# miemie2013/Pytorch-PPYOLO

Measured on AMD Instinct MI355X. Metric: images/sec PPYOLO R50-vd 608x608 bs=8, higher is better.
Workload: dtype f32; 1 GPU; PPYOLO ResNet50-vd (DCNv2, CoordConv, SPP) 608x608, 8 images per GPU, device-resident input -> padded detections; global_batch=8, parallelism=single GPU, hip_graph=True, tile_table=tuned_gfx950_f16x2.json

## Files before the change

include/ppyolo_hip.h:

```cpp
#ifndef PPYOLO_HIP_H_
#define PPYOLO_HIP_H_

#include <stddef.h>
#include <stdint.h>

#ifdef __cplusplus
extern "C" {
#endif

#define PPY_OK 0
#define PPY_ERR_BAD_ARG (-1)
#define PPY_ERR_UNSUPPORTED (-2)
#define PPY_ERR_WORKSPACE (-3)
#define PPY_ERR_LAUNCH (-4)

#define PPY_ACT_NONE 0
#define PPY_ACT_RELU 1
#define PPY_ACT_LEAKY 2

int ppy_version(void);
const char *ppy_error_string(int code);
const char *ppy_last_hip_error(void);
void ppy_note_hip_error(int hip_error);

// ... 161 lines not shown

int ppy_yolo_decode_levels_f32(int nlevels, const float *const *head_out, const int *head_ld, const int *S,
                               const int *downsample, const float *const *h_anchors_px,
                               const int *box_offset, int N, int A, int num_classes, double scale_x_y,
                               int iou_aware, double iou_aware_factor, int clip_bbox, const float *im_size,
                               float *boxes, int M_total, float score_threshold, uint32_t *cand_key,
                               uint32_t *cand_idx, int *cand_count, int cand_cap, void *stream);

size_t ppy_matrix_nms_workspace_bytes(int N);
int ppy_matrix_nms_f32(const float *boxes, int M_total, int num_classes, const uint32_t *cand_key,
                       const uint32_t *cand_idx, const int *cand_count, int cand_cap, int N,
                       float post_threshold, int nms_top_k, int keep_top_k, int use_gaussian,
                       float gaussian_sigma, float *out_dets, int *out_count, int *out_keep_idx,
                       void *ws, size_t ws_bytes, void *stream);
int ppy_nms_candidates_f32(const float *scores, int N, int M, int C, float score_threshold,
                           uint32_t *cand_key, uint32_t *cand_idx, int *cand_count, int cand_cap,
                           void *stream);

int ppy_conv3x3_conv1x1_f32(const float *x_split, int x_ld, const float *xscale, const float *amax_in, const void *wA_f16x2,
                            const float *scaleA_f16x2, const float *shiftA, const void *wB_f16x2, const float *scaleB_f16x2,
                            const float *shiftB, const float *residual, int res_ld, float *y, int y_ld, float *pool, int pool_ld, int N,
                            int H, int W, int CA, int KA, int KB, float t_mul, float t_add, float *amax_out, void *stream);

int ppy_lane_stream_create(void **stream, const uint32_t *h_cu_mask, int mask_words);
int ppy_lane_stream_destroy(void *stream);

#ifdef __cplusplus
}
#endif
#endif
```

pytorch-ppyolo_amd/ppyolo_hip/_lib.py:

```python
import ctypes
import os
from ctypes import c_double, c_float, c_int, c_longlong, c_size_t, c_ulonglong, c_void_p

_HERE = os.path.dirname(os.path.abspath(__file__))
LIB_PATH = os.environ.get('PPYOLO_HIP_LIB') or os.path.join(_HERE, 'lib', 'libppyolo_hip.so')

OK = 0
ACT = {None: 0, 'relu': 1, 'leaky': 2}


class PPYoloHipError(RuntimeError):
    pass


_lib = None

_PROTOS = {
    'ppy_version': (c_int, []),
    'ppy_error_string': (ctypes.c_char_p, [c_int]),
    'ppy_last_hip_error': (ctypes.c_char_p, []),
    'ppy_note_hip_error': (None, [c_int]),
    'ppy_conv2d_split_weights_bf16x3': (c_int, [c_void_p, ctypes.c_longlong, c_void_p, c_void_p]),
    'ppy_conv2d_split_weights_f16x2': (c_int, [c_void_p, c_int, ctypes.c_longlong, c_void_p, c_void_p, c_void_p, c_void_p]),
    'ppy_conv2d_bn_act_f32': (c_int, [c_void_p, c_int, c_void_p, c_void_p, c_void_p, c_void_p, c_void_p, c_void_p, c_void_p,
# ... 65 lines not shown
                            c_void_p]),
    'ppy_dcnv2_sample_f32': (c_int, [c_void_p, c_int, c_void_p, c_int, c_void_p] + [c_int] * 8 + [c_void_p]),
    'ppy_dcnv2_f32': (c_int, [c_void_p, c_int, c_void_p, c_void_p, c_void_p, c_void_p, c_void_p, c_void_p, c_void_p, c_int,
                              c_void_p, c_int] + [c_int] * 10 + [c_void_p, c_void_p, c_void_p, c_size_t, c_void_p]),
    'ppy_dcnv2_workspace_bytes': (c_size_t, [c_int] * 9),
    'ppy_dcnv2_num_configs': (c_int, []),
    'ppy_dcnv2_backward_f32': (c_int, [c_void_p, c_int, c_void_p, c_void_p, c_int, c_void_p, c_int, c_void_p, c_int, c_void_p, c_int, c_void_p]
                               + [c_int] * 7 + [c_void_p, c_size_t, c_void_p]),
    'ppy_dcnv2_backward_workspace_bytes': (c_size_t, [c_int] * 7),
    'ppy_yolo_decode_f32': (c_int, [c_void_p, c_int, c_int, c_int, c_int, c_int, ctypes.POINTER(c_float), c_int,
                                    c_double, c_int, c_double, c_int, c_void_p, c_void_p, c_int, c_int, c_float,
                                    c_void_p, c_void_p, c_void_p, c_int, c_void_p, c_void_p]),
    'ppy_yolo_decode_levels_f32': (c_int, [c_int, c_void_p, c_void_p, c_void_p, c_void_p, c_void_p, c_void_p, c_int, c_int,
                                           c_int, c_double, c_int, c_double, c_int, c_void_p, c_void_p, c_int, c_float,
                                           c_void_p, c_void_p, c_void_p, c_int, c_void_p]),
    'ppy_matrix_nms_f32': (c_int, [c_void_p, c_int, c_int, c_void_p, c_void_p, c_void_p, c_int, c_int, c_float,
                                   c_int, c_int, c_int, c_float, c_void_p, c_void_p, c_void_p, c_void_p, c_size_t,
                                   c_void_p]),
    'ppy_matrix_nms_workspace_bytes': (c_size_t, [c_int]),
    'ppy_nms_candidates_f32': (c_int, [c_void_p, c_int, c_int, c_int, c_float, c_void_p, c_void_p, c_void_p,
                                       c_int, c_void_p]),
    'ppy_conv3x3_conv1x1_f32': (c_int, [c_void_p, c_int, c_void_p, c_void_p, c_void_p, c_void_p, c_void_p, c_void_p, c_void_p, c_void_p, c_void_p,
                                         c_int, c_void_p, c_int, c_void_p, c_int] + [c_int] * 6 + [c_float, c_float, c_void_p, c_void_p]),
    'ppy_lane_stream_create': (c_int, [ctypes.POINTER(c_void_p), ctypes.POINTER(ctypes.c_uint32), c_int]),
    'ppy_lane_stream_destroy': (c_int, [c_void_p]),
}


def exported_symbols():
    return sorted(_PROTOS)


def lib():
    global _lib
    if _lib is None:
        if not os.path.exists(LIB_PATH):
            raise PPYoloHipError(
                'libppyolo_hip.so not found at %s -- build it with `python -c "import __graft_entry__ as g; '
                'g.build()"` (hipcc, gfx950). There is no CPU / PyTorch fallback for the HIP path.' % LIB_PATH)
        import torch
        L = ctypes.CDLL(LIB_PATH)
        for name, (res, args) in _PROTOS.items():
            fn = getattr(L, name)
            fn.restype = res
            fn.argtypes = args
        _lib = L
# ... 10 lines not shown
```

pytorch-ppyolo_amd/ppyolo_hip/csrc/conv_b2b.hip:

```cpp
#include "conv_shared.h"

namespace {

struct B2bArgs {
    const float *x;
    const unsigned short *wA, *wB;
    const float *scaleA, *shiftA, *scaleB, *shiftB;
    const float *res;
    float *y;
    float *pool;
    const float *xscale;
    const float *amax_in;
    float *amax_out;
    float t_mul, t_add;
    int x_ld, res_ld, y_ld, pool_ld, N, H, W, M;
    int skip;
};

template <int CA, int KA, int KB, bool POOL>
__global__ void __launch_bounds__(256, 2) conv_b2b_kernel(const B2bArgs p) {
#if defined(__HIP_DEVICE_COMPILE__)
    constexpr int BM = 128, NW = 4;
    constexpr int TY = 8, TX = 16, WX = TX + 2, WPIX = (TY + 2) * WX;
    constexpr int TNA = KA / 32, HB = KB / 2, TNH = HB / 32;
    constexpr int CCH = CA / 32, NCH = 9 * CCH, KCH = KA / 32;
    constexpr int WIN_CC = WPIX * 128, WIN_BYTES = CCH * WIN_CC;
    constexpr int WIN_UNITS = CCH * WPIX * 8, WIN_PASS = (WIN_UNITS + 64 * NW - 1) / (64 * NW);
    constexpr int B_PASS = (2 * KA) / (16 * NW), G = B_PASS;
    constexpr int BST = 2 * KA * 64, BS_OFF = WIN_PASS * NW * 1024;
    constexpr int A2_BYTES = KCH * BM * 128;
    constexpr int W_OFF = A2_BYTES, W_BYTES = KCH * 2 * HB * 64;
    constexpr int E_OFF = W_OFF + W_BYTES;
    constexpr int B2_PASS = W_BYTES / (1024 * NW);
    static_assert(TY * TX == BM && TY == 2 * NW && TX == 16, "a wave owns two tile rows as eight 2x2 blocks");
    static_assert(KA % 32 == 0 && KB % 64 == 0 && CA % 32 == 0 && (2 * KA) % (16 * NW) == 0 && W_BYTES % (1024 * NW) == 0 && HB % 16 == 0, "shapes");
    static_assert(BS_OFF >= WIN_BYTES && BS_OFF + 3 * BST <= E_OFF + NW * 4096, "window + weight stages fit the allocation");
    typedef __attribute__((address_space(3))) void *lds_ptr;
    extern __shared__ __attribute__((aligned(16))) char smem_b2b[];
    char *smem = smem_b2b;

    const int tid = threadIdx.x, lane = tid & 63;
    const int wave = __builtin_amdgcn_readfirstlane(tid >> 6);
    int tile_id;
    {
        const int nb = (int)gridDim.x, q = nb >> 3, r = nb & 7;
        const int xcd = (int)blockIdx.x & 7, idx = (int)blockIdx.x >> 3;
        tile_id = xcd * q + min(xcd, r) + idx;
    }
    const int hw = p.H * p.W;
    const int tiles_x = (p.W + TX - 1) / TX, tiles_y = (p.H + TY - 1) / TY;
    const int t_n = tile_id / (tiles_x * tiles_y), t_rem = tile_id - t_n * (tiles_x * tiles_y);
    const int t_y = t_rem / tiles_x, t_x = t_rem - t_y * tiles_x;
    const int y0 = t_y * TY, x0 = t_x * TX;
    auto pixel_of = [&](int R) -> int {
        const int w = R >> 5, r = R & 31;
        const int y = y0 + 2 * w + (r >> 4), x = x0 + 2 * (r & 7) + ((r >> 3) & 1);
        return (y < p.H && x < p.W) ? t_n * hw + y * p.W + x : -1;
    };
    const unsigned OOB = 0xFFFFFFF0u;
    {
        const __amdgpu_buffer_rsrc_t rx = __builtin_amdgcn_make_buffer_rsrc((void *)p.x, 0, 0xFFFFFF00u, 0x00020000);
#pragma unroll
        for (int d = 0; d < WIN_PASS; ++d) {
            const int q = (d * NW + wave) * 64 + lane;
            const int pq = q >> 3, cc = pq / WPIX, wp = pq - cc * WPIX;
            const int wy = wp / WX, wx = wp - wy * WX;
            const int y = y0 - 1 + wy, x = x0 - 1 + wx;
            const bool ok = q < WIN_UNITS && (unsigned)y < (unsigned)p.H && (unsigned)x < (unsigned)p.W;
            const unsigned off = ok ? (unsigned)(((t_n * p.H + y) * p.W + x) * (p.x_ld * 4) + cc * 128 + (((q & 7) ^ ((wp >> 1) & 7)) << 4)) : OOB;
            __builtin_amdgcn_raw_ptr_buffer_load_lds(rx, (lds_ptr)(smem + (d * NW + wave) * 1024), 16, off, 0, 0, 0);
        }
    }
    unsigned b_off[B_PASS];
    {
        const int drow = lane >> 2, dslot = lane & 3;
        const long long plane_bytes = (long long)KA * (9 * CA) * 2;
#pragma unroll
        for (int j = 0; j < B_PASS; ++j) {
            const int rb = (j * NW + wave) * 16 + drow;
            const int plane = rb / KA, nrow = rb - plane * KA;
            const int scol = dslot ^ ((rb >> 2) & 3);
            b_off[j] = (unsigned)(plane * plane_bytes + (long long)nrow * 64 + scol * 16);
        }
    }
    const char *wb = reinterpret_cast<const char *>(p.wA);
    auto issue = [&](int stage, int kc) {
        const int cc = kc / 9, tap = kc - cc * 9;
        const long long b_uni = ((long long)tap * CCH + cc) * KA * 64;
        const __amdgpu_buffer_rsrc_t rb = __builtin_amdgcn_make_buffer_rsrc((void *)(wb + b_uni), 0, 0xFFFFFF00u, 0x00020000);
#pragma unroll
        for (int j = 0; j < B_PASS; ++j)
            __builtin_amdgcn_raw_ptr_buffer_load_lds(rb, (lds_ptr)(smem + BS_OFF + stage * BST + (j * NW + wave) * 1024), 16, b_off[j], 0, 0, 0);
    };

    const int frow = lane & 31, fkh = lane >> 5;
    const int wp0 = (2 * wave + (frow >> 4)) * WX + 2 * (frow & 7) + ((frow >> 3) & 1);
    const int a_sw = (frow >> 1) & 7, b_sw = (frow >> 2) & 3;
    int a_foff[2][2], b_foff[2];
#pragma unroll
    for (int s = 0; s < 2; ++s) {
        a_foff[s][0] = frow * 128 + (((2 * s + fkh) ^ a_sw) << 4);
        a_foff[s][1] = frow * 128 + (((4 + 2 * s + fkh) ^ a_sw) << 4);
        b_foff[s] = frow * 64 + (((2 * s + fkh) ^ b_sw) << 4);
    }

    float inv_sa, s2, inv_s2;
    {
        const int n = min(t_n, p.N - 1);
        inv_sa = pow2_inverse(p.xscale[n]);
        s2 = split_scale_of(fmaf(p.t_mul, pow2_above(amax_read(p.amax_in, n)), p.t_add));
        inv_s2 = pow2_inverse(s2);
    }
    issue(0, 0);
    issue(1, 1);
    const int erow = lane >> 3, ec4 = (lane & 7) * 4;
    int pix[4];
#pragma unroll
    for (int t = 0; t < 4; ++t) pix[t] = pixel_of(wave * 32 + erow + 8 * t);
    unsigned roff[4], yoff[4];
#pragma unroll
    for (int t = 0; t < 4; ++t) {
        roff[t] = ((unsigned)max(pix[t], 0) * (unsigned)p.res_ld + (unsigned)ec4) * 4u;
        yoff[t] = ((unsigned)max(pix[t], 0) * (unsigned)p.y_ld + (unsigned)ec4) * 4u;
    }
    const char *res_b = reinterpret_cast<const char *>(p.res);
    constexpr unsigned B2B_OOB = 0x80000000u;
    const __amdgpu_buffer_rsrc_t ry = __builtin_amdgcn_make_buffer_rsrc((void *)p.y, 0, B2B_OOB, 0x00020000);
    const __amdgpu_buffer_rsrc_t rp = __builtin_amdgcn_make_buffer_rsrc((void *)(POOL ? p.pool : p.y), 0, B2B_OOB, 0x00020000);
    const bool no_stores = (p.skip & 4) != 0;
#pragma unroll
    for (int t = 0; t < 4; ++t)
        if (pix[t] < 0 || no_stores) yoff[t] = B2B_OOB;
    floatx4 rv[TNH][4];
    auto load_res = [&](int col0, floatx4 (&dst)[4]) {
#pragma unroll
        for (int t = 0; t < 4; ++t)
            dst[t] = *reinterpret_cast<const floatx4 *>(res_b + (size_t)roff[t] + col0 * 4);
    };
#pragma unroll
    for (int jj = 0; jj < TNH; ++jj) load_res(jj * 32, rv[jj]);
    floatx16 acc[TNA];
#pragma unroll
    for (int j = 0; j < TNA; ++j)
#pragma unroll
        for (int e = 0; e < 16; ++e) acc[j][e] = 0.f;
    if (!(p.skip & 1))
    for (int k = 0; k < NCH; ++k) {
        if (k < 2 && (p.skip & 16))
            wait_vmcnt<0>();
        else if (k < 2)
            wait_vmcnt<G + 4 * TNH>();
        else if (k + 1 < NCH)
            wait_vmcnt<G>();
        else
            wait_vmcnt<0>();
        asm volatile("s_waitcnt lgkmcnt(0)" ::: "memory");
        __builtin_amdgcn_s_barrier();
        if (k + 2 < NCH) issue((k + 2) % 3, k + 2);
        const int st = k % 3;
        const int cc = k / 9, tap = k - cc * 9, tr = tap / 3;
        const int wp = wp0 + tr * WX + (tap - tr * 3);
        const char *a_ptr = smem + cc * WIN_CC + wp * 128;
        const int wsw = (wp >> 1) & 7;
        const char *b_ptr = smem + BS_OFF + st * BST;
#pragma unroll
        for (int s = 0; s < 2; ++s) {
            const uintx4 a0 = *reinterpret_cast<const uintx4 *>(a_ptr + (((2 * s + fkh) ^ wsw) << 4));
            const uintx4 a1 = *reinterpret_cast<const uintx4 *>(a_ptr + (((4 + 2 * s + fkh) ^ wsw) << 4));
            uintx4 b[2][TNA];
#pragma unroll
            for (int pl = 0; pl < 2; ++pl)
#pragma unroll
                for (int j = 0; j < TNA; ++j) b[pl][j] = *reinterpret_cast<const uintx4 *>(b_ptr + (pl * KA + j * 32) * 64 + b_foff[s]);
// ... 6 lines not shown
#pragma unroll
            for (int j = 0; j < TNA; ++j)
                acc[j] = __builtin_amdgcn_mfma_f32_32x32x16_f16(__builtin_bit_cast(f16x8, a0), __builtin_bit_cast(f16x8, b[0][j]), acc[j], 0, 0, 0);
        }
    }
    asm volatile("s_waitcnt lgkmcnt(0)" ::: "memory");
    __builtin_amdgcn_s_barrier();

    const __amdgpu_buffer_rsrc_t rw2 = __builtin_amdgcn_make_buffer_rsrc((void *)p.wB, 0, 0xFFFFFF00u, 0x00020000);
    auto issue_w2 = [&](int half) {
        const int drow = lane >> 2, dslot = lane & 3;
        const unsigned plane_bytes = (unsigned)KB * KA * 2;
#pragma unroll
        for (int j = 0; j < B2_PASS; ++j) {
            const int R = (j * NW + wave) * 16 + drow;
            const int blk = R / HB, r = R - blk * HB;
            const int scol = dslot ^ ((R >> 2) & 3);
            const unsigned off = (unsigned)(blk & 1) * plane_bytes + (unsigned)((blk >> 1) * KB * 64 + (half * HB + r) * 64 + scol * 16);
            __builtin_amdgcn_raw_ptr_buffer_load_lds(rw2, (lds_ptr)(smem + W_OFF + (j * NW + wave) * 1024), 16, off, 0, 0, 0);
        }
    };
    if (p.skip & 1) wait_vmcnt<0>();
    if (p.skip & 2) return;
    issue_w2(0);

    float *sE = reinterpret_cast<float *>(smem + E_OFF) + wave * 1024;
    {
        float rs1[4], rs2[4];
#pragma unroll
        for (int t = 0; t < 4; ++t) {
            rs1[t] = __shfl(inv_sa, (lane >> 3) + 8 * t);
            rs2[t] = __shfl(s2, (lane >> 3) + 8 * t);
        }
#pragma unroll
        for (int j = 0; j < TNA; ++j) {
            const int col = j * 32 + ec4;
            const floatx4 sc = *reinterpret_cast<const floatx4 *>(p.scaleA + col), sh = *reinterpret_cast<const floatx4 *>(p.shiftA + col);
#pragma unroll
            for (int e = 0; e < 16; ++e) {
                const int row = (e & 3) + 8 * (e >> 2) + 4 * (lane >> 5);
                sE[row * 32 + ((lane & 31) ^ ((row & 7) << 2))] = acc[j][e];
            }
            __builtin_amdgcn_wave_barrier();
#pragma unroll
            for (int t = 0; t < 4; ++t) {
                const int rr = erow + 8 * t;
// ... 115 lines not shown
                                       const float *shiftB, const float *residual, int res_ld, float *y, int y_ld, float *pool, int pool_ld,
                                       int N, int H, int W, int CA, int KA, int KB, float t_mul, float t_add, float *amax_out, void *stream) {
    ppy_drop_stale_error();
    PPY_CHECK_ARG(x_split && xscale && amax_in && wA_f16x2 && scaleA_f16x2 && shiftA && wB_f16x2 && scaleB_f16x2 && shiftB && residual && y);
    PPY_CHECK_ARG(N > 0 && H > 0 && W > 0 && t_mul >= 0.f && t_add >= 0.f);
    if (!(CA == 64 && KA == 64 && KB == 256)) return PPY_ERR_UNSUPPORTED;
    PPY_CHECK_ARG(x_ld >= CA && x_ld % 32 == 0 && res_ld >= KB && res_ld % 4 == 0 && y_ld >= KB && y_ld % 4 == 0);
    auto al = [](const void *q) { return ((uintptr_t)q & 15) == 0; };
    PPY_CHECK_ARG(al(x_split) && al(wA_f16x2) && al(wB_f16x2) && al(scaleA_f16x2) && al(shiftA) && al(scaleB_f16x2) && al(shiftB) && al(residual) && al(y));
    if (pool) PPY_CHECK_ARG(H % 2 == 0 && W % 2 == 0 && pool_ld >= KB && pool_ld % 4 == 0 && al(pool));
    const long long M = (long long)N * H * W;
    if (M > 0x7fffffffLL / 4 || (M + W + 1) * x_ld * 4 >= 0xFFFFF000LL || M * res_ld * 4 >= 0xFFFFF000LL || M * y_ld * 4 >= 0x7FFFF000LL ||
        (pool && (M / 4) * pool_ld * 4 >= 0x7FFFF000LL)) return PPY_ERR_UNSUPPORTED;
    B2bArgs a;
    a.x = x_split; a.wA = (const unsigned short *)wA_f16x2; a.wB = (const unsigned short *)wB_f16x2;
    a.scaleA = scaleA_f16x2; a.shiftA = shiftA; a.scaleB = scaleB_f16x2; a.shiftB = shiftB;
    a.res = residual; a.y = y; a.pool = pool; a.xscale = xscale; a.amax_in = amax_in; a.amax_out = amax_out;
    a.t_mul = t_mul; a.t_add = t_add;
    { static const int sk = getenv("PPY_B2B_SKIP") ? atoi(getenv("PPY_B2B_SKIP")) : 0; a.skip = sk; }
    a.x_ld = x_ld; a.res_ld = res_ld; a.y_ld = y_ld; a.pool_ld = pool_ld; a.N = N; a.H = H; a.W = W; a.M = (int)M;
    constexpr size_t lds = 2 * 128 * 128 + 2 * 2 * 128 * 64 + 4 * 4096;
    const unsigned grid = (unsigned)(N * ((H + 7) / 8) * ((W + 15) / 16));
    if (pool) {
        auto k = conv_b2b_kernel<64, 64, 256, true>;
        static PpyLdsAttr attr;
        if (ppy_lds_attr(attr, reinterpret_cast<const void *>(k), (int)lds) != PPY_OK) return PPY_ERR_LAUNCH;
        hipLaunchKernelGGL(k, dim3(grid), dim3(256), lds, (hipStream_t)stream, a);
    } else {
        auto k = conv_b2b_kernel<64, 64, 256, false>;
        static PpyLdsAttr attr;
        if (ppy_lds_attr(attr, reinterpret_cast<const void *>(k), (int)lds) != PPY_OK) return PPY_ERR_LAUNCH;
        hipLaunchKernelGGL(k, dim3(grid), dim3(256), lds, (hipStream_t)stream, a);
    }
    return ppy_launch_status();
}
```

pytorch-ppyolo_amd/ppyolo_hip/engine.py:

```python
import collections
import json
import os

import torch

from . import ops as K
from ._lib import PPYoloHipError

A = collections.namedtuple('A', 'buf coff C N H W')


def fold_bn(bn, bias, K_out, device):
    if bn is not None:
        invstd = 1.0 / torch.sqrt(bn.running_var.detach().float() + bn.eps)
        scale = bn.weight.detach().float() * invstd
        shift = bn.bias.detach().float() - bn.running_mean.detach().float() * scale
        if bias is not None:
            shift = shift + bias.detach().float() * scale
    else:
        scale = torch.ones(K_out, dtype=torch.float32, device=device)
        shift = bias.detach().float().clone() if bias is not None else torch.zeros(K_out, dtype=torch.float32,
                                                                                   device=device)
    return scale.contiguous(), shift.contiguous()

# ... 301 lines not shown
        for b in outs:
            writers.setdefault(b, []).append(op)
    out = []
    for a in ops:
        if a['op'] != 'conv' or not has_f16(a):
            continue
        Ka, R, S, Ca = a['w'].shape
        y = a['y']
        if (R, S, a['stride'], a['pad'], Ca, Ka, a['act']) != (3, 3, 1, 1, 64, 64, 'relu') or a['res'] is not None or a['posb'] is not None \
                or a['ups'] or a.get('pool') is not None or a.get('mpool') is not None or y.buf in pinned \
                or y.coff != 0 or y.C != buffers[y.buf][3] or len(writers.get(y.buf, [])) != 1:
            continue
        rd = readers.get(y.buf, [])
        if len(rd) != 1 or rd[0]['op'] != 'conv':
            continue
        b = rd[0]
        Kb, Rb, Sb, Cb = b['w'].shape
        x = b['x']
        if (Rb, Sb, b['stride'], b['pad'], Cb, Kb, b['act']) != (1, 1, 1, 0, 64, 256, 'relu') or b['res'] is None or b['posb'] is not None \
                or b['ups'] or not has_f16(b) or (x.buf, x.coff, x.C) != (y.buf, 0, 64) or b['res'].buf == y.buf \
                or b.get('stream', 0) != a.get('stream', 0):
            continue
        out.append((a, b))
    return out


class HipExecutor(object):

    def __init__(self, plan, device, use_graph=True, multi_stream=None, share=None):
        if torch.device(device).type != 'cuda':
            raise PPYoloHipError('the HIP executor needs a ROCm device (got %s); there is no CPU path' % device)
        self.plan = plan
        self.device = torch.device(device)
        self.use_graph = use_graph
        self.graph = None
        self._graph_stream = None
        p = plan
        self.bufs = None
        self.x_in = torch.zeros((p.N, 3, p.H, p.W), dtype=torch.float32, device=self.device)
        self.im_size = torch.zeros((p.N, 2), dtype=torch.float32, device=self.device)
        d = p.decode
        if d is not None:
            M, C = d['M_total'], d['num_classes']
            self.boxes = torch.zeros((p.N, M, 4), dtype=torch.float32, device=self.device)
            cap = M * C
            self.cand_key = torch.zeros((p.N, cap), dtype=torch.int32, device=self.device)
# ... 124 lines not shown
    def _split_pairs(self):
        if self.math != 'f16x2' or os.environ.get('PPYOLO_HIP_PRESPLIT', '1') != '1':
            return []
        pinned = {a.buf for a in list(self.plan.head_outs) + list(self.plan.feats)}
        return split_pairs(self.plan.ops, self._op_io, self.plan.buffers, pinned,
                           lambda c: c.get('wf16') is not None and c.get('amax_in_id') is not None,
                           os.environ.get('PPYOLO_HIP_PRESPLIT_3X3_ONLY', '0') == '1')

    def _mark_split_candidates(self):
        for op in self.plan.ops:
            op.pop('gp_in', None)
        for _, cons in self._split_pairs():
            for c in cons:
                c['gp_in'] = True

    def _unlink_splits(self):
        for op in self.plan.ops:
            op.pop('x_split', None)
            op.pop('y_split', None)

    def _link_splits(self, _retry=False):
        if not _retry:
            self._b2b_rejected = set()
        self._unlink_splits()
        self._mark_b2b()
        n = 0
        for pr, cons in self._split_pairs():
            if pr.get('b2b') is not None or pr.get('b2b_of') is not None:
                continue
            if self._split_leaves_launch(pr) or not self._split_capable(pr['cfg'], False) \
                    or any(c.get('b2b') is None and (self._split_leaves_launch(c) or not self._split_capable(c['cfg'], True)) for c in cons):
                continue
            w, sc, sh = pr['w'], pr['scale'], pr['shift']
            l1 = w.abs().double().sum(dim=(1, 2, 3))
            mul = float((sc.abs().double() * l1).max())
            add = sh.abs().double()
            if pr['posb'] is not None:
                pb = self.bufs[pr['posb'].buf].abs().double().reshape(-1, w.shape[0]).amax(dim=0)
                add = add + pb * sc.abs().double()
            add = float(add.max())
            ps = torch.ones(self.plan.N, dtype=torch.float32, device=self.device)
            pr['y_split'] = (ps, mul * (1.0 + 2.0 ** -8), add * (1.0 + 2.0 ** -8) + 1e-30)
            for c in cons:
                c['x_split'] = ps
                n += 1
        undone = False
        for i, op in enumerate(self.plan.ops):
            if op.get('b2b') is not None and op.get('x_split') is None:
                self._b2b_rejected.add(i)
                undone = True
        if undone:
            return self._link_splits(_retry=True)
        return n

    def _unlink_b2b(self):
        for op in self.plan.ops:
            if op.get('b2b') is not None:
                op['b2b'].pop('b2b_of', None)
                op.pop('b2b', None)

    def _mark_b2b(self):
        self._unlink_b2b()
        if self.math != 'f16x2' or os.environ.get('PPYOLO_HIP_B2B', '1') != '1':
            return 0
        pinned = {a.buf for a in list(self.plan.head_outs) + list(self.plan.feats)}
        pairs = b2b_pairs(self.plan.ops, self._op_io, self.plan.buffers, pinned,
                          lambda c: c.get('wf16') is not None and c.get('amax_in_id') is not None)
        rejected = {id(self.plan.ops[i]) for i in getattr(self, '_b2b_rejected', ())}
        pairs = [(a, b) for a, b in pairs if id(a) not in rejected]
        for a, b in pairs:
            if a.get('t_bound') is None:
                w, sc, sh = a['w'], a['scale'], a['shift']
                l1 = w.abs().double().sum(dim=(1, 2, 3))
                a['t_bound'] = (float((sc.abs().double() * l1).max()) * (1.0 + 2.0 ** -8), float(sh.abs().double().max()) * (1.0 + 2.0 ** -8) + 1e-30)
            a['b2b'] = b
            b['b2b_of'] = a
        return len(pairs)

    def presplit_headroom(self):
        out = []
        for op in self.plan.ops:
            ys = op.get('y_split')
# ... 23 lines not shown
            return K.conv2d_workspace_bytes(x.N, x.H, x.W, C, Kout, R, S, op['stride'], op['pad'], op['cfg'],
                                            op['splitk'])
        if op['op'] == 'dcn':
            x = op['x']
            return K.dcnv2_workspace_bytes(x.N, x.H, x.W, x.C, op['w'].shape[0], op['stride'], op['pad'], op['cfg'],
                                           op['splitk'])
        return 0

    def _size_workspace(self):
        need, need_side = 16, 16
        for op in self.plan.setup_ops + self.plan.ops:
            if op.get('stream', 0):
                need_side = max(need_side, self._ws_need(op))
            else:
                need = max(need, self._ws_need(op))
        if self.ws is None or self.ws.numel() * 4 < need:
            self.ws = torch.empty(((need + 3) // 4,), dtype=torch.float32, device=self.device)
        if self.ws_side is None or self.ws_side.numel() * 4 < need_side:
            self.ws_side = torch.empty(((need_side + 3) // 4,), dtype=torch.float32, device=self.device)

    @staticmethod
    def _op_io(op):
        t = op['op']
        if t == 'conv' and op.get('b2b_of') is not None:
            return [], []
        if t == 'conv' and op.get('b2b') is not None:
            b = op['b2b']
            return [op['x'].buf, b['res'].buf], [b['y'].buf] + ([b['pool'].buf] if b.get('pool') is not None else [])
        if t == 'conv':
            ins = [op['x'].buf] + ([op['res'].buf] if op['res'] is not None else [])
            if op.get('mpool') is not None:
                return ins, [op['mpool'].buf]
            return ins, [op['y'].buf] + ([op['pool'].buf] if op.get('pool') is not None else [])
        if t == 'stem':
            return [], [op['y'].buf]
        if t in ('avgpool', 'maxpool') and op.get('owner') is not None:
            return [], []
        if t in ('maxpool', 'avgpool'):
            return [op['x'].buf], [op['y'].buf]
        if t == 'spp':
            return [op['x'].buf], [op['y5'].buf]
        if t == 'dcn':
            return [op['x'].buf, op['om'].buf], [op['y'].buf]
        raise PPYoloHipError('unknown plan op %r' % t)

    def _build_sync_plan(self):
        ops = self.plan.ops
        writers = {}
        self._waits = [[] for _ in ops]
        self._needs_event = set()
        for i, op in enumerate(ops):
            ins, outs = self._op_io(op)
            s = op.get('stream', 0) if self.multi_stream else 0
            for bid in ins:
                for j in writers.get(bid, []):
                    sj = ops[j].get('stream', 0) if self.multi_stream else 0
                    if sj != s and j not in self._waits[i]:
                        self._waits[i].append(j)
                        self._needs_event.add(j)
            for bid in outs:
                writers.setdefault(bid, []).append(i)
        self._side_tail = max([i for i, op in enumerate(ops) if op.get('stream', 0)], default=None) \
            if self.multi_stream else None

    @staticmethod
    def _stream_first():
        return K.stream_first_cfg()

    def _run_op(self, op, ws=None):
        t = op['op']
        ws = self.ws if ws is None else ws
        if t == 'conv' and op.get('b2b_of') is not None:
            return
        if op.get('amax_in2_id') is not None and (t != 'conv' or op.get('b2b') is not None or op.get('mpool') is not None or (
                op.get('pool') is not None and self._stream_first() <= op['cfg'] < self._stream_first() + 2)):
            raise PPYoloHipError('plan op %s reads a buffer with two tracked-maximum blocks through an entry point that takes one' % tune_key(op))
        if t == 'conv' and op.get('b2b') is not None:
            b = op['b2b']
            K.conv3x3_conv1x1(self.view(op['x']), op['x_split'], self._amax(op['amax_in_id']), op['wf16'], op['shift'], b['wf16'], b['shift'],
                              self.view(b['res']), self.view(b['y']), op['t_bound'][0], op['t_bound'][1], self._amax(b.get('amax_out_id')),
                              None if b.get('pool') is None else self.view(b['pool']))
            return
        if t == 'conv' and op.get('pool') is not None and self._stream_first() <= op['cfg'] < self._stream_first() + 2:
            K.conv1x1_expand(self.view(op['x']), op['wf16'], op['shift'], self.view(op['y']), op['act'],
                             None if op['res'] is None else self.view(op['res']), self.view(op['pool']),
                             op['cfg'] - self._stream_first(), self._amax(op.get('amax_in_id')), self._amax(op.get('amax_out_id')))
        elif t == 'conv' and op.get('mpool') is not None:
            K.conv3x3_maxpool(self.view(op['x']), op['wf16'], op['shift'], self.view(op['mpool']), op['act'],
                              self._amax(op.get('amax_in_id')), self._amax(op.get('amax_out_id')))
        elif t == 'conv':
            posb = op['posb']
            K.conv2d_bn_act(self.view(op['x']), op['w'], op['scale'], op['shift'], self.view(op['y']), op['stride'],
                            op['pad'], op['act'], None if op['res'] is None else self.view(op['res']),
                            None if posb is None else self.bufs[posb.buf], op['ups'], op['cfg'], op['splitk'],
                            ws, op.get('w3'), op.get('wf16'), self._amax(op.get('amax_in_id')),
                            self._amax(op.get('amax_out_id')), op.get('posb_f16'), op.get('x_split'), op.get('y_split'),
                            self._amax(op.get('amax_in2_id')))
            if op.get('pool') is not None:
                K.avgpool2x2(self.view(op['y']), self.view(op['pool']))
# ... 331 lines not shown
```

pytorch-ppyolo_amd/ppyolo_hip/ops.py:

```python
import ctypes

import torch

from . import _lib
from ._lib import ACT, check, lib


class View(object):
    __slots__ = ('t', 'coff', 'C')

    def __init__(self, t, coff=0, C=None):
        assert t.dim() == 4 and t.dtype == torch.float32 and t.is_contiguous()
        self.t = t
        self.coff = coff
        self.C = t.shape[3] - coff if C is None else C
        assert 0 <= coff and coff + self.C <= t.shape[3]

    @property
    def N(self):
        return self.t.shape[0]

    @property
    def H(self):
        return self.t.shape[1]
# ... 89 lines not shown
            None if residual is None else residual.ptr, 0 if residual is None else residual.ld,
            _p(posbias), _p(posbias_f16), y.ptr, y.ld, x.N, x.H, x.W, C, K, R, S, stride, pad, ACT[act], int(bool(upsample2x)),
            cfg, splitk, _p(amax_in), _p(amax_out), _p(ws), 0 if ws is None else ws.numel() * ws.element_size(), _stream(),
            _p(x_split), _p(ys), float(ym), float(ya), _p(amax_in2))
        check(rc, 'ppy_conv2d_bn_act_split_f32')
        return
    rc = lib().ppy_conv2d_bn_act_f32(
        x.ptr, x.ld, w_krsc.data_ptr(), _p(w_x3), None if w_f16 is None else w_f16[0].data_ptr(), scale.data_ptr(),
        None if w_f16 is None else w_f16[1].data_ptr(), shift.data_ptr(),
        None if residual is None else residual.ptr, 0 if residual is None else residual.ld,
        _p(posbias), _p(posbias_f16), y.ptr, y.ld, x.N, x.H, x.W, C, K, R, S, stride, pad, ACT[act], int(bool(upsample2x)),
        cfg, splitk, _p(amax_in), _p(amax_out), _p(ws), 0 if ws is None else ws.numel() * ws.element_size(), _stream())
    check(rc, 'ppy_conv2d_bn_act_f32')


def conv3x3_conv1x1(x, x_split, amax_in, wA_f16, shiftA, wB_f16, shiftB, residual, y, t_mul, t_add, amax_out=None, pool=None):
    _dev(x.t, x_split, amax_in, wA_f16[0], wA_f16[1], shiftA, wB_f16[0], wB_f16[1], shiftB, residual.t, y.t)
    KA, KB = shiftA.numel(), shiftB.numel()
    check(lib().ppy_conv3x3_conv1x1_f32(x.ptr, x.ld, x_split.data_ptr(), amax_in.data_ptr(), wA_f16[0].data_ptr(), wA_f16[1].data_ptr(),
                                        shiftA.data_ptr(), wB_f16[0].data_ptr(), wB_f16[1].data_ptr(), shiftB.data_ptr(), residual.ptr,
                                        residual.ld, y.ptr, y.ld, None if pool is None else pool.ptr, 0 if pool is None else pool.ld, x.N, x.H, x.W, x.C, KA, KB,
                                        float(t_mul), float(t_add), _p(amax_out),
                                        _stream()), 'ppy_conv3x3_conv1x1_f32')


def stream_first_cfg():
    return lib().ppy_conv2d_stream_first_config()


def ws_first_cfg():
    return lib().ppy_conv2d_ws_first_config()


def ws_num_cfgs():
    return lib().ppy_conv2d_small_first_config() - lib().ppy_conv2d_ws_first_config()


def small_first_cfg():
    return lib().ppy_conv2d_small_first_config()


def small_num_cfgs():
    return lib().ppy_conv2d_num_configs() - lib().ppy_conv2d_small_first_config()


def patch_first_cfg():
# ... 448 lines not shown
```

Before: 2478 images/s.

## Fuse the 1x1 reduce conv into the 3x3+1x1 back-to-back bottleneck kernel

Adds a bottleneck entry point that computes the leading 1x1 conv (256->64, ReLU) inside the conv3x3+conv1x1 kernel's prologue. The result goes straight into the LDS halo window, so the intermediate activation is never written to or read back from global memory. The planner marks eligible conv->b2b triples and routes them to the fused kernel. In exchange, the halo pixels of the 1x1 conv are recomputed in every tile, the second-stage split scale is taken from a per-wave max, and the kernel's prologue becomes longer and more register-heavy.

```diff
diff --git a/include/ppyolo_hip.h b/include/ppyolo_hip.h
--- a/include/ppyolo_hip.h
+++ b/include/ppyolo_hip.h
@@ -207,6 +207,11 @@
                             const float *shiftB, const float *residual, int res_ld, float *y, int y_ld, float *pool, int pool_ld, int N,
                             int H, int W, int CA, int KA, int KB, float t_mul, float t_add, float *amax_out, void *stream);
 
+int ppy_bottleneck_f32(const float *x, int x_ld, const float *amax_x, const void *w1_f16x2, const float *scale1_f16x2, const float *shift1,
+                       float ys_mul, float ys_add, float *amax_t1, float *yscale1, const void *wA_f16x2, const float *scaleA_f16x2, const float *shiftA,
+                       const void *wB_f16x2, const float *scaleB_f16x2, const float *shiftB, float *y, int y_ld, float *pool, int pool_ld,
+                       int N, int H, int W, int C1, int KA, int KB, float t_mul, float t_add, float *amax_out, void *stream);
+
 int ppy_lane_stream_create(void **stream, const uint32_t *h_cu_mask, int mask_words);
 int ppy_lane_stream_destroy(void *stream);
 
diff --git a/pytorch-ppyolo_amd/ppyolo_hip/_lib.py b/pytorch-ppyolo_amd/ppyolo_hip/_lib.py
--- a/pytorch-ppyolo_amd/ppyolo_hip/_lib.py
+++ b/pytorch-ppyolo_amd/ppyolo_hip/_lib.py
@@ -111,6 +111,8 @@
                                        c_int, c_void_p]),
     'ppy_conv3x3_conv1x1_f32': (c_int, [c_void_p, c_int, c_void_p, c_void_p, c_void_p, c_void_p, c_void_p, c_void_p, c_void_p, c_void_p, c_void_p,
                                          c_int, c_void_p, c_int, c_void_p, c_int] + [c_int] * 6 + [c_float, c_float, c_void_p, c_void_p]),
+    'ppy_bottleneck_f32': (c_int, [c_void_p, c_int, c_void_p, c_void_p, c_void_p, c_void_p, c_float, c_float, c_void_p, c_void_p, c_void_p, c_void_p,
+                                    c_void_p, c_void_p, c_void_p, c_void_p, c_void_p, c_int, c_void_p, c_int] + [c_int] * 6 + [c_float, c_float, c_void_p, c_void_p]),
     'ppy_lane_stream_create': (c_int, [ctypes.POINTER(c_void_p), ctypes.POINTER(ctypes.c_uint32), c_int]),
     'ppy_lane_stream_destroy': (c_int, [c_void_p]),
 }
diff --git a/pytorch-ppyolo_amd/ppyolo_hip/csrc/conv_b2b.hip b/pytorch-ppyolo_amd/ppyolo_hip/csrc/conv_b2b.hip
--- a/pytorch-ppyolo_amd/ppyolo_hip/csrc/conv_b2b.hip
+++ b/pytorch-ppyolo_amd/ppyolo_hip/csrc/conv_b2b.hip
@@ -15,9 +15,17 @@
     float t_mul, t_add;
     int x_ld, res_ld, y_ld, pool_ld, N, H, W, M;
     int skip;
+    const float *x1 = nullptr;
+    const unsigned short *w1 = nullptr;
+    const float *scale1 = nullptr, *shift1 = nullptr;
+    const float *amax_x1 = nullptr;
+    float *amax_t1 = nullptr;
+    float *yscale1 = nullptr;
+    float ys_mul = 0.f, ys_add = 0.f;
+    int x1_ld = 0;
 };
 
-template <int CA, int KA, int KB, bool POOL>
+template <int CA, int KA, int KB, bool POOL, int C1>
 __global__ void __launch_bounds__(256, 2) conv_b2b_kernel(const B2bArgs p) {
 #if defined(__HIP_DEVICE_COMPILE__)
     constexpr int BM = 128, NW = 4;
@@ -58,7 +66,7 @@
         return (y < p.H && x < p.W) ? t_n * hw + y * p.W + x : -1;
     };
     const unsigned OOB = 0xFFFFFFF0u;
-    {
+    if constexpr (C1 == 0) {
         const __amdgpu_buffer_rsrc_t rx = __builtin_amdgcn_make_buffer_rsrc((void *)p.x, 0, 0xFFFFFF00u, 0x00020000);
 #pragma unroll
         for (int d = 0; d < WIN_PASS; ++d) {
@@ -67,7 +75,7 @@
             const int wy = wp / WX, wx = wp - wy * WX;
             const int y = y0 - 1 + wy, x = x0 - 1 + wx;
             const bool ok = q < WIN_UNITS && (unsigned)y < (unsigned)p.H && (unsigned)x < (unsigned)p.W;
-            const unsigned off = ok ? (unsigned)(((t_n * p.H + y) * p.W + x) * (p.x_ld * 4) + cc * 128 + (((q & 7) ^ ((wp >> 1) & 7)) << 4)) : OOB;
+            const unsigned off = ok ? (unsigned)((t_n * p.H + y) * p.W + x) * (unsigned)(p.x_ld * 4) + (unsigned)(cc * 128 + (((q & 7) ^ ((wp >> 1) & 7)) << 4)) : OOB;
             __builtin_amdgcn_raw_ptr_buffer_load_lds(rx, (lds_ptr)(smem + (d * NW + wave) * 1024), 16, off, 0, 0, 0);
         }
     }
@@ -105,15 +113,178 @@
     }
 
     float inv_sa, s2, inv_s2;
-    {
+    floatx4 rv[TNH][4];
+    const int erow = lane >> 3, ec4 = (lane & 7) * 4;
+    if constexpr (C1 == 0) {
         const int n = min(t_n, p.N - 1);
         inv_sa = pow2_inverse(p.xscale[n]);
         s2 = split_scale_of(fmaf(p.t_mul, pow2_above(amax_read(p.amax_in, n)), p.t_add));
         inv_s2 = pow2_inverse(s2);
-    }
-    issue(0, 0);
-    issue(1, 1);
-    const int erow = lane >> 3, ec4 = (lane & 7) * 4;
+        issue(0, 0);
+        issue(1, 1);
+    } else {
+        constexpr int P0_ROWS = 192, P0_A = P0_ROWS * 128, P0_B = 2 * KA * 64, P0_ST = P0_A + P0_B;
+        constexpr int P0_APASS = P0_ROWS * 8 / (64 * NW), P0_BPASS = 2 * KA / (16 * NW), P0_G = P0_APASS + P0_BPASS;
+        constexpr int P0_NCH = C1 / 32;
+        static_assert(KA == 64 && C1 % 32 == 0 && P0_ROWS >= WPIX && P0_ROWS % 32 == 0 && 2 * P0_ST <= E_OFF && (P0_ROWS * 8) % (64 * NW) == 0,
+                      "prologue: two stages below the transposition patches, whole DMA instructions");
+        const int n = min(t_n, p.N - 1);
+        const float sa1 = split_scale_of(amax_read(p.amax_x1, n)), inv_sa1 = pow2_inverse(sa1);
+        const float t1_bound = fmaf(p.ys_mul, 16384.0f * inv_sa1, p.ys_add);
+        const float s1 = split_scale_of(t1_bound);
+        inv_sa = pow2_inverse(s1);
+        s2 = inv_s2 = 1.f;
+        unsigned a1_off[P0_APASS], b1_off[P0_BPASS];
+#pragma unroll
+        for (int j = 0; j < P0_APASS; ++j) {
+            const int row = (j * NW + wave) * 8 + (lane >> 3);
+            const int scol = (lane & 7) ^ ((row >> 1) & 7);
+            const int wy = row / WX, wx = row - wy * WX;
+            const int y = y0 - 1 + wy, x = x0 - 1 + wx;
+            const bool ok = row < WPIX && (unsigned)y < (unsigned)p.H && (unsigned)x < (unsigned)p.W;
+            a1_off[j] = ok ? (unsigned)((t_n * p.H + y) * p.W + x) * (unsigned)(p.x1_ld * 4) + (unsigned)(scol << 4) : OOB;
+        }
+#pragma unroll
+        for (int j = 0; j < P0_BPASS; ++j) {
+            const int rb = (j * NW + wave) * 16 + (lane >> 2);
+            const int plane = rb / KA, nrow = rb - plane * KA;
+            const int scol = (lane & 3) ^ ((rb >> 2) & 3);
+            b1_off[j] = (unsigned)(plane * (KA * C1 * 2) + nrow * 64 + scol * 16);
+        }
+        auto issue1 = [&](int stage, int cc) {
+            const __amdgpu_buffer_rsrc_t ra = __builtin_amdgcn_make_buffer_rsrc((void *)(p.x1 + cc * 32), 0, 0xFFFFFF00u, 0x00020000);
+            const __amdgpu_buffer_rsrc_t rb = __builtin_amdgcn_make_buffer_rsrc((void *)(p.w1 + cc * KA * 32), 0, 0xFFFFFF00u, 0x00020000);
+#pragma unroll
+            for (int j = 0; j < P0_APASS; ++j)
+                __builtin_amdgcn_raw_ptr_buffer_load_lds(ra, (lds_ptr)(smem + stage * P0_ST + (j * NW + wave) * 1024), 16, a1_off[j], 0, 0, 0);
+#pragma unroll
+            for (int j = 0; j < P0_BPASS; ++j)
+                __builtin_amdgcn_raw_ptr_buffer_load_lds(rb, (lds_ptr)(smem + stage * P0_ST + P0_A + (j * NW + wave) * 1024), 16, b1_off[j], 0, 0, 0);
+        };
+        const int rt0 = (3 * wave) >> 1;
+        auto prologue = [&](auto odd_tag) {
+            constexpr int ODD = decltype(odd_tag)::value ? 1 : 0;
+            floatx16 acc1[3];
+#pragma unroll
+            for (int i = 0; i < 3; ++i)
+#pragma unroll
+                for (int e = 0; e < 16; ++e) acc1[i][e] = 0.f;
+            issue1(0, 0);
+            issue1(1, 1);
+            int rwp[4];
+#pragma unroll
+            for (int t = 0; t < 4; ++t) {
+                const int r = erow + 8 * t;
+                rwp[t] = (2 * wave + (r >> 4) + 1) * WX + 2 * (r & 7) + ((r >> 3) & 1) + 1;
+            }
+            static_assert(TNH <= P0_NCH, "the first column half's channels lie in the prologue's chunks");
+#pragma unroll
+            for (int k = 0; k < P0_NCH; ++k) {
+                if (k + 1 < P0_NCH)
+                    wait_vmcnt<P0_G>();
+                else
+                    wait_vmcnt<0>();
+                __builtin_amdgcn_s_barrier();
+                const char *st_ptr = smem + (k & 1) * P0_ST;
+                if (k < TNH) {
+#pragma unroll
+                    for (int t = 0; t < 4; ++t)
+                        rv[k][t] = *reinterpret_cast<const floatx4 *>(st_ptr + rwp[t] * 128 + (((lane & 7) ^ ((rwp[t] >> 1) & 7)) << 4));
+                }
+#pragma unroll
+                for (int s = 0; s < 2; ++s) {
+                    uintx4 a[2][2], b[2][2];
+#pragma unroll
+                    for (int lr = 0; lr < 2; ++lr) {
+                        const char *a_ptr = st_ptr + (rt0 + lr) * 32 * 128 + frow * 128;
+                        const floatx4 lo = *reinterpret_cast<const floatx4 *>(a_ptr + (((4 * s + 2 * fkh) ^ a_sw) << 4));
+                        const floatx4 hi = *reinterpret_cast<const floatx4 *>(a_ptr + (((4 * s + 2 * fkh + 1) ^ a_sw) << 4));
+#pragma unroll
+                        for (int q = 0; q < 4; ++q) {
+                            const float xa = q < 2 ? lo[2 * q] : hi[2 * q - 4], xb = q < 2 ? lo[2 * q + 1] : hi[2 * q - 3];
+                            const unsigned P0 = cvt_pk_f16(xa * sa1, xb * sa1);
+                            a[lr][0][q] = P0;
+                            a[lr][1][q] = cvt_pk_f16(fmaf(xa, sa1, -f16_lo(P0)), fmaf(xb, sa1, -f16_hi(P0)));
+                        }
+                    }
+#pragma unroll
+                    for (int pl = 0; pl < 2; ++pl)
+#pragma unroll
+                        for (int c = 0; c < 2; ++c) b[pl][c] = *reinterpret_cast<const uintx4 *>(st_ptr + P0_A + (pl * KA + c * 32) * 64 + b_foff[s]);
+#pragma unroll
+                    for (int i = 0; i < 3; ++i)
+                        acc1[i] = __builtin_amdgcn_mfma_f32_32x32x16_f16(__builtin_bit_cast(f16x8, a[(i + ODD) >> 1][1]),
+                                                                         __builtin_bit_cast(f16x8, b[0][(i + ODD) & 1]), acc1[i], 0, 0, 0);
+#pragma unroll
+                    for (int i = 0; i < 3; ++i)
+                        acc1[i] = __builtin_amdgcn_mfma_f32_32x32x16_f16(__builtin_bit_cast(f16x8, a[(i + ODD) >> 1][0]),
+                                                                         __builtin_bit_cast(f16x8, b[1][(i + ODD) & 1]), acc1[i], 0, 0, 0);
+#pragma unroll
+                    for (int i = 0; i < 3; ++i)
+                        acc1[i] = __builtin_amdgcn_mfma_f32_32x32x16_f16(__builtin_bit_cast(f16x8, a[(i + ODD) >> 1][0]),
+                                                                         __builtin_bit_cast(f16x8, b[0][(i + ODD) & 1]), acc1[i], 0, 0, 0);
+                }
+                asm volatile("s_waitcnt lgkmcnt(0)" ::: "memory");
+                __builtin_amdgcn_s_barrier();
+                if (k + 2 < P0_NCH) issue1(k & 1, k + 2);
+            }
+            floatx4 sc1[2], sh1[2];
+#pragma unroll
+            for (int c = 0; c < 2; ++c) {
+                sc1[c] = *reinterpret_cast<const floatx4 *>(p.scale1 + c * 32 + ec4);
+                sh1[c] = *reinterpret_cast<const floatx4 *>(p.shift1 + c * 32 + ec4);
+            }
+            issue(0, 0);
+            issue(1, 1);
+            float *sE = reinterpret_cast<float *>(smem + E_OFF) + wave * 1024;
+            float amx1 = 0.f;
+#pragma unroll
+            for (int i = 0; i < 3; ++i) {
+                const int rt = rt0 + ((i + ODD) >> 1), c = (i + ODD) & 1;
+#pragma unroll
+                for (int e = 0; e < 16; ++e) {
+                    const int row = (e & 3) + 8 * (e >> 2) + 4 * (lane >> 5);
+                    sE[row * 32 + ((lane & 31) ^ ((row & 7) << 2))] = acc1[i][e];
+                }
+                __builtin_amdgcn_wave_barrier();
+#pragma unroll
+                for (int t = 0; t < 4; ++t) {
+                    const int rr = erow + 8 * t;
+                    const int wp = rt * 32 + rr;
+                    const int wy = wp / WX, wx = wp - wy * WX;
+                    const int y = y0 - 1 + wy, x = x0 - 1 + wx;
+                    const bool inside = wp < WPIX && (unsigned)y < (unsigned)p.H && (unsigned)x < (unsigned)p.W;
+                    floatx4 v = *reinterpret_cast<const floatx4 *>(sE + rr * 32 + (ec4 ^ ((rr & 7) << 2)));
+#pragma unroll
+                    for (int u = 0; u < 4; ++u) {
+                        v[u] *= inv_sa1;
+                        const float o = fmaf(v[u], sc1[c][u], sh1[c][u]);
+                        v[u] = (inside && o > 0.f) ? o : 0.f;
+                    }
+                    const bool centre = inside && wy >= 1 && wy <= TY && wx >= 1 && wx <= TX;
+                    const float rmx = fmaxf(fmaxf(v[0], v[1]), fmaxf(v[2], v[3]));
+                    amx1 = fmaxf(amx1, centre ? rmx : 0.f);
+                    typedef __attribute__((ext_vector_type(2))) unsigned uintx2_;
+                    const unsigned h0 = cvt_pk_f16(v[0] * s1, v[1] * s1), h1 = cvt_pk_f16(v[2] * s1, v[3] * s1);
+                    const unsigned l0 = cvt_pk_f16(fmaf(v[0], s1, -f16_lo(h0)), fmaf(v[1], s1, -f16_hi(h0)));
+                    const unsigned l1 = cvt_pk_f16(fmaf(v[2], s1, -f16_lo(h1)), fmaf(v[3], s1, -f16_hi(h1)));
+                    if (wp < WPIX) {
+                        char *o2 = smem + c * WIN_CC + wp * 128 + (ec4 & 7) * 2;
+                        const int sw = (wp >> 1) & 7;
+                        *reinterpret_cast<uintx2_ *>(o2 + (((ec4 >> 3) ^ sw) << 4)) = uintx2_{h0, h1};
+                        *reinterpret_cast<uintx2_ *>(o2 + (((4 + (ec4 >> 3)) ^ sw) << 4)) = uintx2_{l0, l1};
+                    }
+                }
+                __builtin_amdgcn_wave_barrier();
+            }
+            if (p.amax_t1) amax_track2(amx1, 0.f, t_n, t_n, p.amax_t1, blockIdx.x * 8 + wave);
+            if (p.yscale1 && tid == 0) p.yscale1[t_n] = s1;
+        };
+        if (wave & 1)
+            prologue(std::true_type());
+        else
+            prologue(std::false_type());
+    }
     int pix[4];
 #pragma unroll
     for (int t = 0; t < 4; ++t) pix[t] = pixel_of(wave * 32 + erow + 8 * t);
@@ -131,14 +302,15 @@
 #pragma unroll
     for (int t = 0; t < 4; ++t)
         if (pix[t] < 0 || no_stores) yoff[t] = B2B_OOB;
-    floatx4 rv[TNH][4];
     auto load_res = [&](int col0, floatx4 (&dst)[4]) {
 #pragma unroll
         for (int t = 0; t < 4; ++t)
             dst[t] = *reinterpret_cast<const floatx4 *>(res_b + (size_t)roff[t] + col0 * 4);
     };
-#pragma unroll
-    for (int jj = 0; jj < TNH; ++jj) load_res(jj * 32, rv[jj]);
+    if constexpr (C1 == 0) {
+#pragma unroll
+        for (int jj = 0; jj < TNH; ++jj) load_res(jj * 32, rv[jj]);
+    }
     floatx16 acc[TNA];
 #pragma unroll
     for (int j = 0; j < TNA; ++j)
@@ -148,7 +320,7 @@
     for (int k = 0; k < NCH; ++k) {
         if (k < 2 && (p.skip & 16))
             wait_vmcnt<0>();
-        else if (k < 2)
+        else if (k < 2 && C1 == 0)
             wait_vmcnt<G + 4 * TNH>();
         else if (k + 1 < NCH)
             wait_vmcnt<G>();
@@ -201,6 +373,19 @@
     };
     if (p.skip & 1) wait_vmcnt<0>();
     if (p.skip & 2) return;
+    if constexpr (C1 > 0) {
+        float mx = 0.f;
+#pragma unroll
+        for (int j = 0; j < TNA; ++j) {
+            const float scj = p.scaleA[j * 32 + (lane & 31)], shj = p.shiftA[j * 32 + (lane & 31)];
+#pragma unroll
+            for (int e = 0; e < 16; ++e) mx = fmaxf(mx, fmaf(acc[j][e] * inv_sa, scj, shj));
+        }
+#pragma unroll
+        for (int o = 32; o > 0; o >>= 1) mx = fmaxf(mx, __shfl_xor(mx, o));
+        s2 = split_scale_of(mx);
+        inv_s2 = pow2_inverse(s2);
+    }
     issue_w2(0);
 
     float *sE = reinterpret_cast<float *>(smem + E_OFF) + wave * 1024;
@@ -362,15 +547,59 @@
     constexpr size_t lds = 2 * 128 * 128 + 2 * 2 * 128 * 64 + 4 * 4096;
     const unsigned grid = (unsigned)(N * ((H + 7) / 8) * ((W + 15) / 16));
     if (pool) {
-        auto k = conv_b2b_kernel<64, 64, 256, true>;
+        auto k = conv_b2b_kernel<64, 64, 256, true, 0>;
         static PpyLdsAttr attr;
         if (ppy_lds_attr(attr, reinterpret_cast<const void *>(k), (int)lds) != PPY_OK) return PPY_ERR_LAUNCH;
         hipLaunchKernelGGL(k, dim3(grid), dim3(256), lds, (hipStream_t)stream, a);
     } else {
-        auto k = conv_b2b_kernel<64, 64, 256, false>;
+        auto k = conv_b2b_kernel<64, 64, 256, false, 0>;
         static PpyLdsAttr attr;
         if (ppy_lds_attr(attr, reinterpret_cast<const void *>(k), (int)lds) != PPY_OK) return PPY_ERR_LAUNCH;
         hipLaunchKernelGGL(k, dim3(grid), dim3(256), lds, (hipStream_t)stream, a);
     }
     return ppy_launch_status();
 }
+
+extern "C" int ppy_bottleneck_f32(const float *x, int x_ld, const float *amax_x, const void *w1_f16x2, const float *scale1_f16x2,
+                                  const float *shift1, float ys_mul, float ys_add, float *amax_t1, float *yscale1, const void *wA_f16x2,
+                                  const float *scaleA_f16x2, const float *shiftA, const void *wB_f16x2, const float *scaleB_f16x2,
+                                  const float *shiftB, float *y, int y_ld, float *pool, int pool_ld, int N, int H, int W, int C1, int KA,
+                                  int KB, float t_mul, float t_add, float *amax_out, void *stream) {
+    ppy_drop_stale_error();
+    PPY_CHECK_ARG(x && amax_x && w1_f16x2 && scale1_f16x2 && shift1 && wA_f16x2 && scaleA_f16x2 && shiftA && wB_f16x2 && scaleB_f16x2 && shiftB && y);
+    PPY_CHECK_ARG(N > 0 && H > 0 && W > 0 && t_mul >= 0.f && t_add >= 0.f && ys_mul >= 0.f && ys_add >= 0.f);
+    if (!(C1 == 256 && KA == 64 && KB == 256)) return PPY_ERR_UNSUPPORTED;
+    PPY_CHECK_ARG(x_ld >= C1 && x_ld % 4 == 0 && y_ld >= KB && y_ld % 4 == 0);
+    auto al = [](const void *q) { return ((uintptr_t)q & 15) == 0; };
+    PPY_CHECK_ARG(al(x) && al(w1_f16x2) && al(scale1_f16x2) && al(shift1) && al(wA_f16x2) && al(wB_f16x2) && al(scaleA_f16x2) && al(shiftA) &&
+                  al(scaleB_f16x2) && al(shiftB) && al(y));
+    if (pool) PPY_CHECK_ARG(H % 2 == 0 && W % 2 == 0 && pool_ld >= KB && pool_ld % 4 == 0 && al(pool));
+    const long long M = (long long)N * H * W;
+    if (M > 0x7fffffffLL / 4 || M * x_ld * 4 >= 0xFFFFF000LL || M * y_ld * 4 >= 0x7FFFF000LL ||
+        (pool && (M / 4) * pool_ld * 4 >= 0x7FFFF000LL)) return PPY_ERR_UNSUPPORTED;
+    B2bArgs a;
+    a.x = nullptr; a.xscale = nullptr; a.amax_in = nullptr; a.x_ld = 0;
+    a.wA = (const unsigned short *)wA_f16x2; a.wB = (const unsigned short *)wB_f16x2;
+    a.scaleA = scaleA_f16x2; a.shiftA = shiftA; a.scaleB = scaleB_f16x2; a.shiftB = shiftB;
+    a.res = x; a.y = y; a.pool = pool; a.amax_out = amax_out;
+    a.t_mul = t_mul; a.t_add = t_add;
+    { static const int sk = getenv("PPY_B2B_SKIP") ? atoi(getenv("PPY_B2B_SKIP")) : 0; a.skip = sk; }
+    a.res_ld = x_ld; a.y_ld = y_ld; a.pool_ld = pool_ld; a.N = N; a.H = H; a.W = W; a.M = (int)M;
+    a.x1 = x; a.w1 = (const unsigned short *)w1_f16x2; a.scale1 = scale1_f16x2; a.shift1 = shift1; a.amax_x1 = amax_x; a.amax_t1 = amax_t1;
+    a.yscale1 = yscale1;
+    a.ys_mul = ys_mul; a.ys_add = ys_add; a.x1_ld = x_ld;
+    constexpr size_t lds = 2 * 128 * 128 + 2 * 2 * 128 * 64 + 4 * 4096;
+    const unsigned grid = (unsigned)(N * ((H + 7) / 8) * ((W + 15) / 16));
+    if (pool) {
+        auto k = conv_b2b_kernel<64, 64, 256, true, 256>;
+        static PpyLdsAttr attr;
+        if (ppy_lds_attr(attr, reinterpret_cast<const void *>(k), (int)lds) != PPY_OK) return PPY_ERR_LAUNCH;
+        hipLaunchKernelGGL(k, dim3(grid), dim3(256), lds, (hipStream_t)stream, a);
+    } else {
+        auto k = conv_b2b_kernel<64, 64, 256, false, 256>;
+        static PpyLdsAttr attr;
+        if (ppy_lds_attr(attr, reinterpret_cast<const void *>(k), (int)lds) != PPY_OK) return PPY_ERR_LAUNCH;
+        hipLaunchKernelGGL(k, dim3(grid), dim3(256), lds, (hipStream_t)stream, a);
+    }
+    return ppy_launch_status();
+}
diff --git a/pytorch-ppyolo_amd/ppyolo_hip/engine.py b/pytorch-ppyolo_amd/ppyolo_hip/engine.py
--- a/pytorch-ppyolo_amd/ppyolo_hip/engine.py
+++ b/pytorch-ppyolo_amd/ppyolo_hip/engine.py
@@ -347,6 +347,35 @@
                 or b.get('stream', 0) != a.get('stream', 0):
             continue
         out.append((a, b))
+    return out
+
+
+def block_triples(ops, op_io, buffers, pinned, pairs, has_f16):
+    readers, writers = {}, {}
+    for op in ops:
+        ins, outs = op_io(op)
+        for b in ins:
+            readers.setdefault(b, []).append(op)
+        for b in outs:
+            writers.setdefault(b, []).append(op)
+    out = []
+    for a, b in pairs:
+        ws_ = writers.get(a['x'].buf, [])
+        if len(ws_) != 1 or ws_[0]['op'] != 'conv':
+            continue
+        c = ws_[0]
+        K1, R, S, C1 = c['w'].shape
+        y, x, res = c['y'], c['x'], b['res']
+        if (R, S, c['stride'], c['pad'], C1, K1, c['act']) != (1, 1, 1, 0, 256, 64, 'relu') or c['res'] is not None or c['posb'] is not None \
+                or c['ups'] or c.get('pool') is not None or c.get('mpool') is not None or not has_f16(c) or c.get('amax_in2_id') is not None \
+                or y.buf in pinned or y.coff != 0 or y.C != buffers[y.buf][3] or (a['x'].buf, a['x'].coff, a['x'].C) != (y.buf, 0, 64) \
+                or res is None or (x.buf, x.coff, x.C) != (res.buf, res.coff, res.C) \
+                or not (c.get('stream', 0) == a.get('stream', 0) == b.get('stream', 0)):
+            continue
+        rd = readers.get(y.buf, [])
+        if len(rd) != 1 or rd[0] is not a:
+            continue
+        out.append((c, a, b))
     return out
 
 
@@ -517,6 +546,7 @@
     def _link_splits(self, _retry=False):
         if not _retry:
             self._b2b_rejected = set()
+        self._unlink_blocks()
         self._unlink_splits()
         self._mark_b2b()
         n = 0
@@ -546,13 +576,37 @@
                 undone = True
         if undone:
             return self._link_splits(_retry=True)
+        self._mark_blocks()
         return n
 
     def _unlink_b2b(self):
+        self._unlink_blocks()
         for op in self.plan.ops:
             if op.get('b2b') is not None:
                 op['b2b'].pop('b2b_of', None)
                 op.pop('b2b', None)
+
+    def _unlink_blocks(self):
+        for op in self.plan.ops:
+            op.pop('blk', None)
+            op.pop('blk_of', None)
+
+    def _mark_blocks(self):
+        self._unlink_blocks()
+        if self.math != 'f16x2' or os.environ.get('PPYOLO_HIP_B2B', '1') != '1' or os.environ.get('PPYOLO_HIP_BLOCK', '1') != '1':
+            return 0
+        pinned = {a.buf for a in list(self.plan.head_outs) + list(self.plan.feats)}
+        pairs = [(a, a['b2b']) for a in self.plan.ops if a.get('b2b') is not None and a.get('x_split') is not None]
+        triples = block_triples(self.plan.ops, self._op_io, self.plan.buffers, pinned, pairs,
+                                lambda c: c.get('wf16') is not None and c.get('amax_in_id') is not None)
+        n = 0
+        for c, a, b in triples:
+            if c.get('y_split') is None or a['x_split'] is not c['y_split'][0]:
+                continue
+            a['blk'] = c
+            c['blk_of'] = a
+            n += 1
+        return n
 
     def _mark_b2b(self):
         self._unlink_b2b()
@@ -622,8 +676,11 @@
     @staticmethod
     def _op_io(op):
         t = op['op']
-        if t == 'conv' and op.get('b2b_of') is not None:
+        if t == 'conv' and (op.get('b2b_of') is not None or op.get('blk_of') is not None):
             return [], []
+        if t == 'conv' and op.get('blk') is not None:
+            b = op['b2b']
+            return [op['blk']['x'].buf], [b['y'].buf] + ([b['pool'].buf] if b.get('pool') is not None else [])
         if t == 'conv' and op.get('b2b') is not None:
             b = op['b2b']
             return [op['x'].buf, b['res'].buf], [b['y'].buf] + ([b['pool'].buf] if b.get('pool') is not None else [])
@@ -670,11 +727,20 @@
     def _run_op(self, op, ws=None):
         t = op['op']
         ws = self.ws if ws is None else ws
-        if t == 'conv' and op.get('b2b_of') is not None:
+        if t == 'conv' and (op.get('b2b_of') is not None or op.get('blk_of') is not None):
             return
         if op.get('amax_in2_id') is not None and (t != 'conv' or op.get('b2b') is not None or op.get('mpool') is not None or (
                 op.get('pool') is not None and self._stream_first() <= op['cfg'] < self._stream_first() + 2)):
             raise PPYoloHipError('plan op %s reads a buffer with two tracked-maximum blocks through an entry point that takes one' % tune_key(op))
+        if t == 'conv' and op.get('blk') is not None:
+            c, b = op['blk'], op['b2b']
+            if c.get('amax_in2_id') is not None:
+                raise PPYoloHipError('plan op %s reads a buffer with two tracked-maximum blocks through an entry point that takes one' % tune_key(c))
+            K.bottleneck(self.view(c['x']), self._amax(c['amax_in_id']), c['wf16'], c['shift'], c['y_split'][1], c['y_split'][2],
+                         op['wf16'], op['shift'], b['wf16'], b['shift'], self.view(b['y']), op['t_bound'][0], op['t_bound'][1],
+                         self._amax(c.get('amax_out_id')), self._amax(b.get('amax_out_id')), None if b.get('pool') is None else self.view(b['pool']),
+                         c['y_split'][0])
+            return
         if t == 'conv' and op.get('b2b') is not None:
             b = op['b2b']
             K.conv3x3_conv1x1(self.view(op['x']), op['x_split'], self._amax(op['amax_in_id']), op['wf16'], op['shift'], b['wf16'], b['shift'],
diff --git a/pytorch-ppyolo_amd/ppyolo_hip/ops.py b/pytorch-ppyolo_amd/ppyolo_hip/ops.py
--- a/pytorch-ppyolo_amd/ppyolo_hip/ops.py
+++ b/pytorch-ppyolo_amd/ppyolo_hip/ops.py
@@ -135,6 +135,19 @@
                                         residual.ld, y.ptr, y.ld, None if pool is None else pool.ptr, 0 if pool is None else pool.ld, x.N, x.H, x.W, x.C, KA, KB,
                                         float(t_mul), float(t_add), _p(amax_out),
                                         _stream()), 'ppy_conv3x3_conv1x1_f32')
+
+
+def bottleneck(x, amax_x, w1_f16, shift1, ys_mul, ys_add, wA_f16, shiftA, wB_f16, shiftB, y, t_mul, t_add, amax_t1=None, amax_out=None,
+               pool=None, yscale1=None):
+    _dev(x.t, amax_x, w1_f16[0], w1_f16[1], shift1, wA_f16[0], wA_f16[1], shiftA, wB_f16[0], wB_f16[1], shiftB, y.t)
+    K1, KA, KB = shift1.numel(), shiftA.numel(), shiftB.numel()
+    if K1 != KA:
+        raise _lib.PPYoloHipError('bottleneck: conv1 has %d output channels, conv2 reads %d' % (K1, KA))
+    check(lib().ppy_bottleneck_f32(x.ptr, x.ld, amax_x.data_ptr(), w1_f16[0].data_ptr(), w1_f16[1].data_ptr(), shift1.data_ptr(),
+                                   float(ys_mul), float(ys_add), _p(amax_t1), _p(yscale1), wA_f16[0].data_ptr(), wA_f16[1].data_ptr(), shiftA.data_ptr(),
+                                   wB_f16[0].data_ptr(), wB_f16[1].data_ptr(), shiftB.data_ptr(), y.ptr, y.ld,
+                                   None if pool is None else pool.ptr, 0 if pool is None else pool.ld, x.N, x.H, x.W, x.C, KA, KB,
+                                   float(t_mul), float(t_add), _p(amax_out), _stream()), 'ppy_bottleneck_f32')
 
 
 def stream_first_cfg():
```

After: 2506 images/s, median of 6. 1.01x the previous value.
